# twesterhout/distributed-matvec

Measured on AMD Instinct MI355X. Metric: matvecs/sec, higher is better.
Workload: dtype f64; 1 GPU; heisenberg_chain_32: y <- H x, 601080390 basis states, 9927521280 off-diagonal non-zeros, f64 vectors, sigma/x/y resident in HBM; partitions=1, partitioning=single, exchange=none, kernel=direct-pull+staged, x=u(hash(sigma, 42)) - 0.5, exchange_bytes_per_matvec=0

## Files before the change

distributed-matvec_amd/_lib.py:

```python
from __future__ import annotations

import ctypes as C
import os

_HERE = os.path.dirname(os.path.abspath(__file__))
LIB_PATH = os.path.join(_HERE, os.environ.get("LS_AMD_LIB", "libls_amd.so"))

c_u64p = C.POINTER(C.c_uint64)
c_i64p = C.POINTER(C.c_int64)
c_f64p = C.POINTER(C.c_double)
c_intp = C.POINTER(C.c_int)


class ChplExternalArray(C.Structure):

    _fields_ = [("elts", C.c_void_p), ("num_elts", C.c_uint64), ("freer", C.c_void_p)]


class LsHsBasis(C.Structure):

    _fields_ = [
        ("number_sites", C.c_int),
        ("number_particles", C.c_int),
        ("number_up", C.c_int),
# ... 224 lines not shown
        "ls_amd_repl_plan": (vp, [vp]),
        "ls_amd_repl_exchange_bytes": (C.c_int64, [vp]),
        "ls_amd_repl_x_in_bytes": (C.c_int64, [vp]),
        "ls_amd_enumerate_states": (C.c_int, [bp, C.c_int, C.POINTER(vp), C.POINTER(vp), c_i64p, vp]),
        "ls_amd_gather": (C.c_int, [C.c_int64, vp, C.c_int, C.c_int, vp, vp, vp]),
        "ls_amd_mask_counts": (C.c_int, [C.c_int64, vp, C.c_int, c_i64p, vp]),
        "ls_amd_block_to_hashed": (C.c_int, [C.c_int64, vp, C.c_int, C.c_int, vp, C.POINTER(vp), vp]),
        "ls_amd_hashed_to_block": (C.c_int, [C.c_int64, vp, C.c_int, C.c_int, C.POINTER(vp), vp, vp]),
        "ls_amd_basis_group_order": (C.c_int, [bp]),
        "ls_amd_basis_apply_group_element": (C.c_uint64, [bp, C.c_int, C.c_uint64]),
        "ls_amd_basis_group_character": (C.c_int, [bp, C.c_int, c_f64p, c_f64p]),
        "ls_amd_test_tilemap": (C.c_int64, [C.c_int64, C.c_int, C.c_int64, C.POINTER(C.POINTER(C.c_uint64))]),
        "ls_amd_test_window_find": (C.c_int, [C.POINTER(C.c_uint64), C.c_int, C.c_uint64]),
        "ls_amd_test_nw_find": (C.c_int, [C.POINTER(C.c_uint64), C.c_int, C.c_uint64]),
        "ls_amd_test_chain_near_table": (C.c_int, [C.c_int, C.c_int, C.POINTER(C.c_int16)]),
        "ls_amd_test_rep_trivial_dihedral": (C.c_uint64, [C.c_uint64, C.c_int, C.c_int, C.c_int]),
        "ls_amd_bench_k4": (C.c_int, [C.c_int, C.c_int, C.c_int, C.c_int, C.c_int64, vp, vp, vp]),
        "ls_amd_test_free": (None, [vp]),
        "ls_amd_test_translation_cosets": (C.c_int, [bp, C.POINTER(C.c_int)]),
        "ls_amd_test_rep_by_cosets": (C.c_uint64, [bp, C.c_uint64]),
        "ls_amd_test_d4_mask": (C.c_int, [bp]),
        "ls_amd_test_gtab_bits": (C.c_int, [C.c_int, C.c_int64]),
        "ls_amd_test_gtab_build": (C.c_int, [C.c_int, C.c_int, C.c_int64, C.POINTER(C.c_uint64), C.POINTER(C.c_uint32), C.POINTER(C.POINTER(C.c_uint64))]),
        "ls_amd_test_gtab_find": (C.c_int64, [C.c_int, C.c_int, C.POINTER(C.c_uint64), C.c_uint64]),
        "ls_amd_test_primme_comminfo_offset": (C.c_int, []),
        "ls_amd_test_primme_sumtype_offset": (C.c_int, []),
        "ls_amd_test_primme_nlocal_offset": (C.c_int, []),
        "ls_amd_test_primme_matrix_offset": (C.c_int, []),
        "ls_hs_init": (None, []),
        "ls_hs_exit": (None, []),
# ... 84 lines not shown
```

distributed-matvec_amd/csrc/host.c:

```c
#define _GNU_SOURCE
#include <math.h>
#include <pthread.h>
#include <stdarg.h>
#include <stdio.h>
#include <stdlib.h>
#include <string.h>

#include "../../include/ls_amd.h"
#include "../../include/ls_chpl.h"
#include "../../include/ls_hs.h"
#include "lsk.h"

static __thread char g_last_error[1024] = "";
static ls_amd_error_handler g_handler = NULL;

static int set_error(char const *fmt, ...) {
    va_list ap;
    va_start(ap, fmt);
    vsnprintf(g_last_error, sizeof(g_last_error), fmt, ap);
    va_end(ap);
    return -1;
}
static int dev_error(void) { return set_error("%s", lsk_last_error()); }
int ls_amd_internal_error(char const *fmt, ...) {
// ... 1561 lines not shown
    void *d_tilemap;
    int has_pairs;
    int has_push_staged;
    int one_rank_full_basis;
    lsk_pairplan pairs;
    void *d_pair_recs, *d_rank_low, *d_pair_binom, *d_states32, *d_pair_rows, *d_pair_sites;
    int global_index;
    int has_hubbard;
    lsk_hubbard hubbard;
    void *d_hub[6];
    int has_chain;
    int chain_cached;
    void *d_chain_cache;
    int chain_wide;
    uint64_t *d_chain_rec;
    double chain_v[2];
    int64_t chain_row0;
    void *d_htab;
    uint32_t *d_slot_of;
    int htab_bits;
    void *d_xs;
    int pull_halo;
    int idx_mode;
    struct ls_amd_gtab *gtab;
    uint64_t *d_vtab;
    int64_t row_g0;
    lsk_pullbuf pbuf;
    int64_t split_rows;
    int64_t split_active;
    int slot_cache, slot_cache_valid;
// ... 533 lines not shown
    int const L = NBITS(op->basis);
    int const inv = op->basis->spin_inversion != 0;
    if (inv && (pl->dbs.proj != LSK_PROJ_INVERSION || pl->family != FAMILY_DIRECT_PULL || (L & 1) || BEXT(op->basis)->hamming_weight != L / 2)) return 0;
    if (L > 64 || (!inv && pl->dbs.proj != LSK_PROJ_NONE) ||
        !ext->is_real || !ext->is_hermitian || ext->runs.n_runs <= 0 || ext->n_diag <= 0)
        return 0;
    int extra = 0;
    if (inv) for (int q = 0; q < ext->runs.n_runs; ++q) if (ext->runs.lo0[q] + ext->runs.cnt[q] - 1 == L - 2) extra = 1;
    if (ext->n_groups - ext->runs.n_run_groups + extra > 2) return 0;
    for (int g = ext->runs.n_run_groups; g < ext->n_groups; ++g) {
        lsk_group const *G = &ext->groups[g];
        if (G->fast != LSK_GROUP_EXCHANGE || G->v_im != 0.0 || __builtin_popcountll(G->x) != 2) return 0;
    }
    return 1;
}
static int setup_chain(ls_amd_plan *pl, lsk_index index, int64_t n, uint64_t const *d_reps, void *stream) {
    struct ls_amd_operator_ext const *ext = OEXT(pl->op);
    int nc = ext->n_groups - ext->runs.n_run_groups;
    int const Ls = NBITS(pl->op->basis);
    int const inv = pl->dbs.proj == LSK_PROJ_INVERSION;
    uint64_t const top = 1ULL << (Ls - 1);
    uint64_t cx[3];
    double cv[3];
    int k = 0;
    if (inv)
        for (int q = 0; q < pl->dop.runs.n_runs; ++q)
            if (pl->dop.runs.lo0[q] + pl->dop.runs.cnt[q] - 1 == Ls - 2) {
                cx[k] = 3ULL << (Ls - 2);
                cv[k++] = pl->dop.runs.v_re[q] * (double)pl->op->basis->spin_inversion;
                if (--pl->dop.runs.cnt[q] == 0) {
// ... 36 lines not shown
        pl->chain_v[1] = nc > 1 ? cv[1] : 0.0;
    }
    if (build_tilemap(pl, n, lsk_chain_tile_rows(pl->cplx)) != 0) return -1;
    if (!pl->cplx && NBITS(pl->op->basis) <= 32 && !pl->chain_wide && n > 0) {
        void *q;
        if (lsk_malloc(&q, sizeof(uint64_t) * (size_t)n) != 0) {
            if (pl->d_chain_cache) { lsk_free(pl->d_chain_cache); pl->d_chain_cache = NULL; }
            if (pl->d_tilemap) { lsk_free(pl->d_tilemap); pl->d_tilemap = NULL; memset(&pl->tilemap, 0, sizeof(pl->tilemap)); }
            pl->chain_cached = 0;
            return 0;
        }
        pl->d_chain_rec = (uint64_t *)q;
        DEV(lsk_chain_pack(n, d_reps, pl->chain_cached ? pl->d_chain_cache : NULL, (uint64_t *)q, stream));
        DEV(lsk_sync(stream));
        if (pl->chain_cached <= 1 && pl->d_chain_cache) { lsk_free(pl->d_chain_cache); pl->d_chain_cache = NULL; }
    }
    pl->has_chain = 1;
    return 0;
}

static int pair_cmp(void const *pa, void const *pb) {
    lsk_pair const *a = (lsk_pair const *)pa, *b = (lsk_pair const *)pb;
    int const ca = a->j < 11 ? 0 : (a->i < 11 ? 1 : 2), cb = b->j < 11 ? 0 : (b->i < 11 ? 1 : 2);
    if (ca != cb) return ca - cb;
    if (a->i != b->i) return (int)a->i - (int)b->i;
    return (int)a->j - (int)b->j;
}
static int setup_pairs(ls_amd_plan *pl, int64_t n, uint64_t const *d_reps, void *stream) {
    ls_hs_operator const *op = pl->op;
    struct ls_amd_operator_ext const *ext = OEXT(op);
// ... 814 lines not shown
            if (ps->d_ttab) lsk_free(ps->d_ttab);
            if (ps->d_soff) lsk_free(ps->d_soff);
            if (ps->scatter_gt) ls_amd_internal_gtab_release(ps->scatter_gt);
            free(ps->h_soff);
            free(ps->ttab_first);
            free(ps->send_counts); free(ps->h_beta_off); free(ps->h_val_off);
        }
        free(pl->parts);
    }
    if (pl->d_gtable) lsk_free(pl->d_gtable);
    if (pl->d_row_gidx) lsk_free(pl->d_row_gidx);
    if (pl->d_norms_global) lsk_free(pl->d_norms_global);
    if (pl->d_tilemap) lsk_free(pl->d_tilemap);
    if (pl->d_chain_cache) lsk_free(pl->d_chain_cache);
    if (pl->d_chain_rec) lsk_free(pl->d_chain_rec);
    if (pl->d_pair_recs) lsk_free(pl->d_pair_recs);
    for (int k = 0; k < 6; ++k) if (pl->d_hub[k]) lsk_free(pl->d_hub[k]);
    if (pl->d_pair_rows) lsk_free(pl->d_pair_rows);
    if (pl->d_pair_sites) lsk_free(pl->d_pair_sites);
    if (pl->d_rank_low) lsk_free(pl->d_rank_low);
    if (pl->d_pair_binom) lsk_free(pl->d_pair_binom);
    if (pl->d_states32) lsk_free(pl->d_states32);
    if (pl->d_htab) lsk_free(pl->d_htab);
    if (pl->d_slot_of) lsk_free(pl->d_slot_of);
    if (pl->d_xs) lsk_free(pl->d_xs);
    if (pl->gtab) ls_amd_internal_gtab_release(pl->gtab);
    split_free(pl);
    block_free(pl);
    if (pl->d_send) lsk_free(pl->d_send);
    if (pl->d_cursors) lsk_free(pl->d_cursors);
// ... 141 lines not shown
    if (rc) { lsk_free(nrm); return dev_error(); }
    *d_norms = (double *)nrm;
    return 0;
}

int ls_amd_matvec_replicated(ls_amd_plan *pl, void const *d_x_global, void *d_y_local, void *stream) {
    part_state *ps = &pl->parts[0];
    int slot;
    ls_amd_internal_count_matvec(pl);
    if (pl->family == FAMILY_REPL_DIRECT) {
        int const st = stage_begin(pl, ST_ROWS, stream);
        slot = timing_begin(pl, stream);
        if (pl->has_chain)
            DEV(lsk_chain(pl->dop, pl->dbs, pl->gindex, pl->cplx, pl->chain_wide, pl->d_chain_rec != NULL, pl->tilemap, ps->count,
                          pl->d_chain_rec ? pl->d_chain_rec : ps->d_reps, pl->chain_row0, pl->gindex.count, d_x_global, d_y_local,
                          pl->chain_cached, pl->d_chain_cache, pl->chain_v[0], pl->chain_v[1], stream));
        else
            DEV(lsk_direct_gx(pl->dop, pl->dbs, pl->gindex, pl->cplx, pl->tilemap, ps->d_reps, pl->d_row_gidx, d_x_global,
                          d_y_local, pl->d_err, stream));
        timing_end(pl, slot, stream);
        stage_end(pl, st, stream);
        return 0;
    }
    if (pl->family == FAMILY_REPL_TILE && pl->idx_mode) {
        lsk_pullidx ix;
        ix.tab = pl->gtab->tab;
        ix.perm = pl->gtab->d_perm;
        ix.row_g0 = pl->row_g0;
        ix.vtab = NULL;
        int const st = stage_begin(pl, ST_ROWS, stream);
        slot = timing_begin(pl, stream);
// ... 90 lines not shown
    case FAMILY_DIRECT_PULL:
        if (pl->has_hubbard) return "direct-pull+hubbard";
        return pl->has_chain ? "direct-pull+staged" : pl->has_pairs ? (pl->pairs.sites ? "direct-pull+pairsites" : pl->pairs.rows ? "direct-pull+pairrows" : "direct-pull+pairs") : "direct-pull";
    case FAMILY_TILE_PULL: return pl->idx_mode ? (pl->slot_cache ? "tile-pull+indexed+cached" : (pl->d_vtab ? "tile-pull+values" : "tile-pull+indexed")) : "tile-pull";
    case FAMILY_REPL_DIRECT:
        return pl->has_chain ? "replicated-direct-pull+staged" : "replicated-direct-pull";
    case FAMILY_REPL_TILE: return pl->idx_mode ? (pl->slot_cache ? "replicated-tile-pull+indexed+cached" : "replicated-tile-pull+indexed") : "replicated-tile-pull";
    default: return pl->streams ? "tile+streams" : (pl->has_push_staged ? "tile(one rank: push+staged)" : "tile");
    }
}
int ls_amd_plan_packet_bytes(ls_amd_plan const *pl) { return pl->key_bytes + (pl->cplx ? 16 : 8); }
int ls_amd_plan_row_bytes(ls_amd_plan const *pl) {
    if (pl->has_hubbard) return 0;
    if (pl->has_pairs) return pl->pairs.wide ? 8 : 4;
    if (pl->has_chain) {
        if (pl->d_chain_rec) return 8;
        int const narrow = NBITS(pl->op->basis) <= 32 && !pl->chain_wide;
        return (narrow ? 4 : 8) + pl->chain_cached * (pl->chain_wide ? 8 : 4);
    }
    if (pl->family == FAMILY_TILE_PULL || pl->family == FAMILY_REPL_TILE) return 16;
    return 8;
}
int64_t ls_amd_plan_nnz(ls_amd_plan const *pl) { return pl->nnz; }
int ls_amd_plan_send_counts(ls_amd_plan const *pl, int round, int64_t *counts) {
    if (pl->family != FAMILY_TILE) { for (int d = 0; d < pl->P; ++d) counts[d] = 0; return 0; }
    part_state const *ps = &pl->parts[0];
    if (round < 0 || round >= ps->rounds) return set_error("round out of range");
    memcpy(counts, ps->send_counts + (size_t)round * pl->P, sizeof(int64_t) * pl->P);
    return 0;
}

// ... 240 lines not shown
        }
    } else if (pl->family != FAMILY_DIRECT_PULL) {
        int const st = stage_begin(pl, ST_DIAG, stream);
        for (int p = 0; p < pl->n_local; ++p)
            DEV(lsk_diag(pl->dop, pl->cplx, pl->parts[p].count, pl->parts[p].d_reps, d_x[p], d_y[p], stream));
        stage_end(pl, st, stream);
    }
    if (pl->dop.n_groups == 0 && pl->family != FAMILY_DIRECT_PULL) return 0;
    if (pl->family != FAMILY_TILE) {
        part_state *ps = &pl->parts[0];
        int const st = stage_begin(pl, ST_ROWS, stream);
        int slot = timing_begin(pl, stream);
        if (pl->has_chain)
            DEV(lsk_chain(pl->dop, pl->dbs, ps->index, pl->cplx, pl->chain_wide, pl->d_chain_rec != NULL, pl->tilemap, ps->count,
                          pl->d_chain_rec ? pl->d_chain_rec : ps->d_reps, 0, ps->count, d_x[0], d_y[0], pl->chain_cached,
                          pl->d_chain_cache, pl->chain_v[0], pl->chain_v[1], stream));
        else if (pl->has_pairs)
            DEV(lsk_pairs(pl->pairs, pl->dbs.hamming_weight, pl->cplx, pl->tilemap, ps->count, d_x[0], d_y[0], stream));
        else if (pl->has_hubbard)
            DEV(lsk_hubbard_apply(pl->hubbard, pl->dop, pl->cplx, pl->tilemap, d_x[0], d_y[0], stream));
        else if (pl->has_push_staged)
            DEV(lsk_push_staged(pl->dop, pl->dbs, ps->index, pl->cplx, pl->tilemap, ps->count, ps->d_reps, d_x[0], d_y[0], pl->d_err, stream));
        else
            DEV(lsk_direct(pl->dop, pl->dbs, ps->index, pl->cplx, pl->family == FAMILY_DIRECT_PULL ? (OEXT(pl->op)->is_hermitian ? 1 : 2) : 0, pl->tilemap, ps->d_reps,
                           d_x[0], d_y[0], pl->d_err, stream));
        timing_end(pl, slot, stream);
        stage_end(pl, st, stream);
        return 0;
    }
    int const P = pl->P;
    if (pl->streams) {
// ... 2537 lines not shown
```

distributed-matvec_amd/csrc/k_rows.hip:

```cpp
#include <hip/hip_runtime.h>
#include "lsk_dev.hpp"

template <bool CPLX>
__global__ __launch_bounds__(kBlock) void k_diag(lsk_runs runs, int n_diag, lsk_term const *__restrict__ diag,
                                                 int64_t n, uint64_t const *__restrict__ reps,
                                                 double const *__restrict__ x, double *__restrict__ y) {
    for (int64_t i = (int64_t)blockIdx.x * kBlock + threadIdx.x; i < n; i += (int64_t)gridDim.x * kBlock) {
        uint64_t a = reps[i];
        double dr, di;
        diag_coeff<uint64_t, false>(runs, n_diag, diag, a, dr, di);
        if (CPLX) {
            double xr = x[2 * i], xi = x[2 * i + 1];
            y[2 * i] = dr * xr - di * xi;
            y[2 * i + 1] = dr * xi + di * xr;
        } else {
            y[i] = dr * x[i];
        }
    }
}

extern "C" int lsk_diag(lsk_operator op, int cplx, int64_t n, uint64_t const *reps, void const *x, void *y,
                        void *stream) {
    if (n == 0 || op.n_diag == 0) return 0;
    dim3 g(grid_for(n)), b(kBlock);
// ... 521 lines not shown
    } else if (cplx) hipLaunchKernelGGL((k_push_t<uint64_t, true, 512>), g, b, 0, (hipStream_t)stream, LSK_PT_ARGS);
    else hipLaunchKernelGGL((k_push_t<uint64_t, false, 1024>), g, b, 0, (hipStream_t)stream, LSK_PT_ARGS);
#undef LSK_PT_ARGS
    LSK_LAUNCH_CHECK();
    return 0;
}

extern "C" int lsk_direct_gx(lsk_operator op, lsk_basis bs, lsk_index ix, int cplx, lsk_tilemap tm, uint64_t const *reps,
                             int64_t const *row_gidx, void const *x_global, void *y, int *d_err, void *stream) {
    return direct_dispatch(op, bs, ix, cplx, 1, tm, reps, x_global, y, d_err, stream, 1, row_gidx);
}

constexpr int kChainHalo = 512;
constexpr int kChainLdsPairs = 12;
constexpr int kChainFar = 12;

__device__ __forceinline__ double cx_load_nt(double const *p) { return __builtin_nontemporal_load(p); }
__device__ __forceinline__ double2 cx_load_nt(double2 const *p) {
    typedef double d2v __attribute__((ext_vector_type(2)));
    const d2v v = __builtin_nontemporal_load(reinterpret_cast<d2v const *>(p));
    return make_double2(v.x, v.y);
}
constexpr int kChainFarC = 6;

template <typename W, typename R, bool CPLX, int TILE, bool REC>
__global__ __launch_bounds__(kBlock, (CPLX || sizeof(R) == 8 ? 5 : (sizeof(W) == 8 ? 6 : 7))) void k_chain_t(lsk_runs runs, int n_diag, lsk_term const *__restrict__ diag,
                                                    int hamming_weight, uint4 const *__restrict__ g_img, int img16, int kc,
                                                    int near_off,
                                                    uint64_t const *__restrict__ tilemap, int64_t slots_per_xcd, int64_t n,
                                                    uint64_t const *__restrict__ reps, void const *__restrict__ x_v,
                                                    void *__restrict__ y_v, int hb, int n_cached,
                                                    R const *__restrict__ cache, double cv0, double cv1, int64_t row0,
                                                    int64_t n_x) {
    typedef typename ChainX<CPLX>::type X;
    typedef WordTraits<W> WT;
    constexpr int NB = ChainTraits<W, R>::NB;
    constexpr int HALO = CPLX ? 256 : kChainHalo;
    constexpr int LDSP = CPLX ? 11 : kChainLdsPairs;
    constexpr int WINDOW = TILE + 2 * HALO + 2;
    constexpr int FAR = CPLX ? kChainFarC : kChainFar;
    constexpr R kNone = ~(R)0;
    X const *__restrict__ x = (X const *)x_v;
    X *__restrict__ y = (X *)y_v;
    const bool extra_stream = kAblate && (n_cached & 0x100);
    const int nt_from = !kAblate ? 99 : ((n_cached & 0x200) ? 20 : ((n_cached & 0x400) ? 0 : 99));
    if (kAblate) n_cached &= 0xff;
    uint64_t ex_next = 0;
    extern __shared__ uint4 s_img[];
    R const *const s_binom = reinterpret_cast<R const *>(s_img);
    uint2 const *const s_near = reinterpret_cast<uint2 const *>(reinterpret_cast<char const *>(s_img) + near_off);
    __shared__ X s_x[WINDOW + 1];
    for (int k = threadIdx.x; k < img16; k += kBlock) s_img[k] = g_img[k];
    (void)NB;
    if (threadIdx.x == 0) s_x[WINDOW] = cx_zero<X>();
    const int xcd = blockIdx.x & 7;
    const int64_t blocks_per_xcd = gridDim.x >> 3;
    const int lane = threadIdx.x & 63;
    tilemap += (int64_t)xcd * slots_per_xcd;
    uint32_t const *__restrict__ reps32 = reinterpret_cast<uint32_t const *>(reps);
    for (int64_t t = blockIdx.x >> 3; t < slots_per_xcd; t += blocks_per_xcd) {
        const uint64_t slot = tilemap[t];
        const int cnt = (int)(slot >> 48);
        if (cnt == 0) continue;
        const int64_t i0 = (int64_t)(slot & 0xffffffffffffULL);
        const int64_t w0 = (row0 + i0 - HALO) & ~(int64_t)1;
        W a_next = 0;
        R t0_next = kNone, t1_next = kNone;
        auto load_row = [&](int64_t row, W &a_out, R &t0_out, R &t1_out) {
            if (REC) {
                const uint64_t rec = __builtin_nontemporal_load(reps + row);
                a_out = (W)(uint32_t)rec;
                t0_out = (R)(uint32_t)(rec >> 32);
                if (n_cached == 0) t0_out = kNone;
            } else {
                if (sizeof(W) == 4) a_out = (W)__builtin_nontemporal_load(reps32 + 2 * row);
                else a_out = (W)__builtin_nontemporal_load(reps + row);
                if (n_cached > 0) t0_out = __builtin_nontemporal_load(cache + row);
            }
            if (n_cached > 1) t1_out = __builtin_nontemporal_load(cache + (size_t)n + (size_t)row);
            if (kAblate && extra_stream) ex_next = __builtin_nontemporal_load(reps + (row < (n >> 1) ? row + (n >> 1) : row - (n >> 1)));
        };
        const int wave0 = (int)(threadIdx.x & ~63u);
        if (wave0 < cnt) {
            const int64_t rr = i0 + ((int)threadIdx.x < cnt ? (int)threadIdx.x : cnt - 1);
            load_row(rr, a_next, t0_next, t1_next);
        }
        __syncthreads();
        if (CPLX) {
            for (int j = threadIdx.x; j < WINDOW; j += kBlock) {
                const int64_t row = w0 + j;
                s_x[j] = (row >= 0 && row < n_x) ? x[row] : cx_zero<X>();
            }
        } else {
            double const *xd = (double const *)x_v;
            double *sd = (double *)s_x;
            for (int j = 2 * threadIdx.x; j < WINDOW; j += 2 * kBlock) {
                const int64_t row = w0 + j;
                double2 v;
                if (row >= 0 && row + 1 < n_x) v = *reinterpret_cast<double2 const *>(xd + row);
                else { v.x = (row >= 0 && row < n_x) ? xd[row] : 0.0; v.y = (row + 1 >= 0 && row + 1 < n_x) ? xd[row + 1] : 0.0; }
                sd[j] = v.x;
                sd[j + 1] = v.y;
            }
        }
        __syncthreads();
        const int own0 = (int)(row0 + i0 - w0);
        X y_pending = cx_zero<X>();
        int64_t i_pending = -1;
#pragma unroll 1
        for (int sub = 0; sub < TILE / kBlock; ++sub) {
            const int r = sub * kBlock + threadIdx.x;
            if (i_pending >= 0) cx_store_nt(y + i_pending, y_pending);
            i_pending = -1;
            const W a = a_next;
            const R t0 = t0_next, t1 = t1_next;
            const uint64_t ex = ex_next;
            if (sub + 1 < TILE / kBlock && (sub + 1) * kBlock + wave0 < cnt) {
                const int64_t in = i0 + (r + kBlock < cnt ? r + kBlock : cnt - 1);
                load_row(in, a_next, t0_next, t1_next);
            }
            if (sub * kBlock + wave0 >= cnt) continue;
            const bool ghost = r >= cnt;
            const int64_t i = i0 + (ghost ? cnt - 1 : r);
            const R ig = (R)(row0 + i);
            X g0 = cx_zero<X>(), g1 = cx_zero<X>();
            if (n_cached > 0) g0 = x[t0 != kNone ? t0 : ig];
            if (n_cached > 1) g1 = x[t1 != kNone ? t1 : ig];
            const int jr = own0 + (int)(i - i0);
            const X xr = s_x[jr];
            double dr, di;
            diag_coeff<W, true>(runs, n_diag, diag, a, dr, di);
            X acc = cx_scale(dr, xr);
            const W tdiff = a ^ (a >> 1);
            const W a0 = readfirstlane_t<W>(a);
            const W adiff = a0 ^ readlane_t<W>(a, 63);
            const int ubit = adiff == 0 ? 0 : (int)(8 * sizeof(W)) - (sizeof(W) == 4 ? __clz((int)(uint32_t)adiff) : __clzll((long long)(uint64_t)adiff));
            const R ig0 = readfirstlane_t<R>(ig);
            const uint32_t dl = (uint32_t)(ig - ig0);
            for (int q = 0; q < runs.n_runs; ++q) {
                const int lo0 = runs.lo0[q];
                int lo_end = lo0 + runs.cnt[q];
                const double vr = runs.v_re[q];
                int k = WT::popc(a & (W)(((uint64_t)1 << lo0) - 1));
                int lo = lo0;
                const int e1 = lo_end < LDSP ? lo_end : LDSP;
                const int near_end = lo0 > e1 ? lo0 : e1;
                int split = hb == 0 ? lo_end : (hb < near_end ? near_end : (hb > lo_end ? lo_end : hb));
                if (hb != 0 && split < ubit) split = ubit < lo_end ? ubit : lo_end;
                const bool uni = split < lo_end;
                unsigned long long m = 0;
                R off = 0;
// ... 79 lines not shown
#pragma unroll 4
                for (; lo < lo_end; ++lo) {
                    const bool bit = (a >> lo) & 1;
                    const bool act = (tdiff >> lo) & 1;
                    const R d = s_binom[lo * kc + k];
                    k += bit ? 1 : 0;
                    R idx = bit ? (R)(ig + d) : (R)(ig - d);
                    idx = act ? idx : ig;
                    cx_fma(act ? vr : 0.0, x[idx], acc);
                }
            }
            cx_fma(t0 != kNone ? cv0 : 0.0, g0, acc);
            cx_fma(t1 != kNone ? cv1 : 0.0, g1, acc);
            if (kAblate && extra_stream && ex == 0x0123456789abcdefULL) cx_fma(1.0, xr, acc);
            y_pending = acc;
            i_pending = ghost ? -1 : i;
        }
        if (i_pending >= 0) cx_store_nt(y + i_pending, y_pending);
    }
}

template <typename W, typename R>
__global__ __launch_bounds__(kBlock) void k_chain_cache(int64_t n, uint64_t const *__restrict__ reps, uint64_t xmask, uint64_t inv_mask,
                                                        int hamming_weight, uint64_t const *__restrict__ g_binom,
                                                        R *__restrict__ out, int *__restrict__ flag) {
    constexpr int NB = ChainTraits<W, R>::NB;
    __shared__ R s_binom[NB * LSK_BINOM_K];
    for (int k = threadIdx.x; k < NB * LSK_BINOM_K; k += blockDim.x) s_binom[k] = (R)g_binom[k];
    __syncthreads();
    for (int64_t i = (int64_t)blockIdx.x * kBlock + threadIdx.x; i < n; i += (int64_t)gridDim.x * kBlock) {
        const W a = (W)reps[i];
        R t = ~(R)0;
        if (WordTraits<W>::popc(a & (W)xmask) == 1) {
// ... 20 lines not shown
    LSK_LAUNCH_CHECK();
    return 0;
}

__global__ __launch_bounds__(kBlock) void k_chain_pack(int64_t n, uint64_t const *__restrict__ reps,
                                                       uint32_t const *__restrict__ cache, uint64_t *__restrict__ out) {
    for (int64_t i = (int64_t)blockIdx.x * kBlock + threadIdx.x; i < n; i += (int64_t)gridDim.x * kBlock)
        out[i] = (uint64_t)(uint32_t)reps[i] | ((uint64_t)(cache ? cache[i] : 0xffffffffu) << 32);
}
extern "C" int lsk_chain_pack(int64_t n, uint64_t const *reps, void const *cache, uint64_t *out, void *stream) {
    if (n == 0) return 0;
    hipLaunchKernelGGL(k_chain_pack, dim3(grid_for(n)), dim3(kBlock), 0, (hipStream_t)stream, n, reps, (uint32_t const *)cache, out);
    LSK_LAUNCH_CHECK();
    return 0;
}

__global__ void k_binom_narrow(uint64_t const *__restrict__ in, uint32_t *__restrict__ out, int n) {
    for (int k = blockIdx.x * blockDim.x + threadIdx.x; k < n; k += gridDim.x * blockDim.x) out[k] = (uint32_t)in[k];
}
template <typename R> static R const *chain_binom(uint64_t const *g_binom, hipStream_t stream);
template <> uint64_t const *chain_binom<uint64_t>(uint64_t const *g_binom, hipStream_t) { return g_binom; }
template <> uint32_t const *chain_binom<uint32_t>(uint64_t const *g_binom, hipStream_t stream) {
    static uint64_t const *src = nullptr;
    static uint32_t *narrow = nullptr;
    static std::mutex lock;
    std::lock_guard<std::mutex> guard(lock);
    if (src != g_binom || !narrow) {
        if (!narrow && hipMalloc((void **)&narrow, sizeof(uint32_t) * 64 * LSK_BINOM_K) != hipSuccess) return nullptr;
        hipLaunchKernelGGL(k_binom_narrow, dim3(4), dim3(kBlock), 0, stream, g_binom, narrow, 64 * LSK_BINOM_K);
        src = g_binom;
// ... 50 lines not shown
            if (rsize == 4) reinterpret_cast<uint32_t *>(img.data())[n * kc + k] = (uint32_t)C[n][k];
            else reinterpret_cast<uint64_t *>(img.data())[n * kc + k] = C[n][k];
        }
    if (chain_near_fill(C, elem, ldsp, reinterpret_cast<int16_t *>(img.data() + near_off)) != 0) return -1;
    ChainImage c = {rsize, rows, kc, elem, ldsp, device, nullptr, bytes, near_off};
    if (hipMalloc((void **)&c.dev, (size_t)bytes) != hipSuccess) { snprintf(g_err, sizeof(g_err), "chain_lds_image: no device memory"); return -1; }
    if (hipMemcpy(c.dev, img.data(), (size_t)bytes, hipMemcpyHostToDevice) != hipSuccess) { (void)hipFree(c.dev); snprintf(g_err, sizeof(g_err), "chain_lds_image: copy failed"); return -1; }
    cache.push_back(c);
    *out = c;
    return 0;
}

template <typename W, typename R, bool CPLX, int TILE, bool REC>
static int launch_chain(lsk_operator op, lsk_basis bs, lsk_index ix, lsk_tilemap tm, int64_t n, uint64_t const *reps,
                        int64_t row0, int64_t n_x, void const *x, void *y, int n_cached, void const *cache, double cv0,
                        double cv1, void *stream) {
    int64_t gb = tm.slots_per_xcd * 8;
    ChainImage img;
    if (chain_lds_image((int)sizeof(R), ChainTraits<W, R>::NB, bs.hamming_weight, CPLX ? 16 : 8, CPLX ? 11 : kChainLdsPairs, &img) != 0) return -1;
    hipLaunchKernelGGL((k_chain_t<W, R, CPLX, TILE, REC>), dim3((unsigned)gb), dim3(kBlock), (size_t)img.bytes, (hipStream_t)stream, op.runs,
                       op.n_diag, op.diag, bs.hamming_weight, img.dev, img.bytes / 16, img.kc, img.near_off, tm.entries, tm.slots_per_xcd, n, reps, x, y,
                       kChainLdsPairs, n_cached | ((kAblate && (bs.debug_ablate & 128)) ? 0x100 : 0) | ((kAblate && (bs.debug_ablate & 4096)) ? 0x200 : 0) |
                           ((kAblate && (bs.debug_ablate & 8192)) ? 0x400 : 0), (R const *)cache, cv0, cv1, row0, n_x);
    LSK_LAUNCH_CHECK();
    return 0;
}

extern "C" int lsk_chain_tile_rows(int cplx) { return cplx ? 512 : 1024; }

extern "C" int lsk_chain(lsk_operator op, lsk_basis bs, lsk_index ix, int cplx, int wide_ranks, int fused_records, lsk_tilemap tm,
                         int64_t n, uint64_t const *reps, int64_t row0, int64_t n_x, void const *x, void *y, int n_cached,
                         void const *cache, double cv0, double cv1, void *stream) {
    if (n == 0 || tm.slots_per_xcd == 0) return 0;
    const bool narrow = bs.number_sites <= 32 && !wide_ranks;
#define LSK_CHAIN_ARGS op, bs, ix, tm, n, reps, row0, n_x, x, y, n_cached, cache, cv0, cv1, stream
    if (fused_records) {
        if (!narrow || cplx) { snprintf(g_err, sizeof(g_err), "lsk_chain: fused records need 32-bit states and ranks and f64 vectors"); return -1; }
        return launch_chain<uint32_t, uint32_t, false, 1024, true>(LSK_CHAIN_ARGS);
    }
    if (narrow) {
        if (!cplx) { snprintf(g_err, sizeof(g_err), "lsk_chain: 32-bit states and ranks with f64 vectors run on fused records (lsk_chain_pack)"); return -1; }
        return launch_chain<uint32_t, uint32_t, true, 512, false>(LSK_CHAIN_ARGS);
    }
    if (!wide_ranks) return cplx ? launch_chain<uint64_t, uint32_t, true, 512, false>(LSK_CHAIN_ARGS) : launch_chain<uint64_t, uint32_t, false, 1024, false>(LSK_CHAIN_ARGS);
    return cplx ? launch_chain<uint64_t, uint64_t, true, 512, false>(LSK_CHAIN_ARGS) : launch_chain<uint64_t, uint64_t, false, 1024, false>(LSK_CHAIN_ARGS);
#undef LSK_CHAIN_ARGS
}

constexpr int kPairLowBits = 11;
constexpr int kPairHalo = 512;
// ... 463 lines not shown
```

distributed-matvec_amd/csrc/lsk.h:

```cpp
#ifndef LSK_H
#define LSK_H

#include <stddef.h>
#include <stdint.h>

#ifdef __cplusplus
extern "C" {
#endif

#define LSK_BENES_STAGES 11
#define LSK_BINOM_K 34
#define LSK_MAX_PARTS 256

typedef struct lsk_term {
    double v_re, v_im;
    uint64_t m, r, s;
} lsk_term;

enum { LSK_GROUP_GENERIC = 0, LSK_GROUP_EXCHANGE = 1,
       LSK_GROUP_HOP_LO = 2, LSK_GROUP_HOP_HI = 3 };

typedef struct lsk_group {
    uint64_t x;
    double v_re, v_im;
// ... 149 lines not shown
int lsk_event_create(void **ev);
int lsk_event_destroy(void *ev);
int lsk_event_record(void *ev, void *stream);
int lsk_event_elapsed_ms(void *start, void *stop, float *ms);

int lsk_fill_random(int64_t n, uint64_t const *states, uint64_t seed, int cplx, void *out, void *stream);

int lsk_diag(lsk_operator op, int cplx, int64_t n, uint64_t const *reps, void const *x, void *y,
             void *stream);
int lsk_direct_validate(lsk_operator op, lsk_basis bs, lsk_index ix, int64_t n, uint64_t const *reps, int *d_err, void *stream);
int lsk_direct(lsk_operator op, lsk_basis bs, lsk_index ix, int cplx, int pull, lsk_tilemap tm,
               uint64_t const *reps, void const *x, void *y, int *d_err, void *stream);
int lsk_chain_tile_rows(int cplx);
int lsk_chain(lsk_operator op, lsk_basis bs, lsk_index ix, int cplx, int wide_ranks, int fused_records, lsk_tilemap tm,
              int64_t n, uint64_t const *reps, int64_t row0, int64_t n_x, void const *x, void *y, int n_cached,
              void const *cache, double cv0, double cv1, void *stream);
#define LSK_MAX_PAIRS 128
#define LSK_PAIR_KC 20
typedef struct lsk_pair {
    uint8_t i, j, pad[6];
    double v;
    double vz;
} lsk_pair;
typedef struct lsk_pair_row {
    uint64_t between;
    double v, vz;
    int i, j;
} lsk_pair_row;
#define LSK_PAIR_SITE_MAX_DEGREE 8
#define LSK_PAIR_SITE_MAX_CLASSES 64
typedef struct lsk_pairplan {
// ... 17 lines not shown
typedef struct lsk_species {
    int64_t n;
    int deg;
    uint32_t const *words;
    uint32_t const *rank;
    double const *coef;
} lsk_species;
typedef struct lsk_hubbard {
    int L, cplx_coef;
    lsk_species up, dn;
} lsk_hubbard;
int lsk_hubbard_apply(lsk_hubbard hb, lsk_operator op, int cplx, lsk_tilemap tm, void const *x, void *y, void *stream);
int lsk_narrow_states(int64_t n, uint64_t const *reps, uint32_t *out, void *stream);

int lsk_chain_pack(int64_t n, uint64_t const *reps, void const *cache, uint64_t *out, void *stream);
int lsk_chain_cache(lsk_basis bs, lsk_index ix, int64_t n, uint64_t const *reps, uint64_t xmask, void *out, int wide_ranks,
                    int *d_flag, void *stream);
int lsk_tile(lsk_operator op, lsk_basis bs, lsk_index ix, int cplx, int count_only, int P, int me,
             int64_t row0, int64_t row1, uint64_t const *reps, double const *norms, void const *x,
             void *y, unsigned long long *d_cursors, lsk_round_layout const *d_layout, void *d_send,
             unsigned long long *d_counts, int *d_err, void *stream);
int lsk_tile_wv_max_parts(void);
int lsk_tile_wv(lsk_operator op, lsk_basis bs, lsk_index ix, lsk_gdir gd, int cplx, int count_only, int P, int me,
                int64_t row0, int64_t row1, uint64_t const *reps, double const *norms, void const *x, void *y,
                uint32_t *d_wtab, lsk_round_layout const *d_layout, void *d_send, int *d_err, lsk_gtab own_gt, void *stream);
int lsk_tile_st_max_classes(void);
int lsk_tile_st(lsk_operator op, lsk_gdir gd, uint64_t const *d_binom, int cplx, int count_only, int P, int S, int tile_rows,
                int64_t row0, int64_t row1, uint64_t const *reps, void const *x, uint32_t *d_ttab,
                lsk_round_layout const *d_layout, void *d_send, int *d_err, void *stream);
typedef struct lsk_wsrc {
// ... 290 lines not shown
```

include/ls_amd.h:

```cpp
#ifndef LS_AMD_H
#define LS_AMD_H

#include "ls_hs.h"

#ifdef __cplusplus
extern "C" {
#endif

typedef enum { LS_AMD_F64 = 0, LS_AMD_C128 = 1 } ls_amd_dtype;

typedef enum {
    LS_AMD_MODE_AUTO = 0,
    LS_AMD_MODE_PUSH = 1,
    LS_AMD_MODE_PULL = 2
} ls_amd_mode;

typedef struct ls_amd_plan ls_amd_plan;

char const *ls_amd_last_error(void);
typedef void (*ls_amd_error_handler)(char const *message);
void ls_amd_set_error_handler(ls_amd_error_handler handler);

int ls_amd_device_count(void);
int ls_amd_set_device(int device);
// ... 232 lines not shown
                                   uint64_t *x, uint64_t *s);

int ls_amd_basis_group_order(ls_hs_basis const *basis);
int ls_amd_basis_fermion_signs(ls_hs_basis const *basis);
int ls_amd_test_fermion_sign(ls_hs_basis const *basis, int element, uint64_t state, int table);
int ls_amd_basis_spin_flip(ls_hs_basis const *basis);
int ls_amd_test_group_element_kind(ls_hs_basis const *basis, int element);
uint64_t ls_amd_basis_apply_group_element(ls_hs_basis const *basis, int element, uint64_t state);
int ls_amd_basis_group_character(ls_hs_basis const *basis, int element, double *re, double *im);

int64_t ls_amd_test_tilemap(int64_t n, int tile_rows, int64_t chunk, uint64_t **entries);
void ls_amd_test_free(void *p);
int ls_amd_test_window_find(uint64_t const *reps, int n, uint64_t key);
int ls_amd_test_nw_find(uint64_t const *reps, int n, uint64_t key);
int ls_amd_test_chain_near_table(int elem, int ldsp, int16_t *out);
uint64_t ls_amd_test_rep_trivial_dihedral(uint64_t a, int L, int inv, int reflect);
int ls_amd_bench_k4(int L, int inv, int reflect, int variant, int64_t n, uint64_t const *d_reps, uint64_t *d_out, void *stream);
int ls_amd_test_translation_cosets(ls_hs_basis const *basis, int *n_cosets);
uint64_t ls_amd_test_rep_by_cosets(ls_hs_basis const *basis, uint64_t state);
int ls_amd_test_d4_mask(ls_hs_basis const *basis);
int ls_amd_test_gtab_bits(int L, int64_t n);
int ls_amd_test_gtab_build(int L, int bbits, int64_t n, uint64_t const *reps, uint32_t const *payload, uint64_t **entries);
int64_t ls_amd_test_gtab_find(int L, int bbits, uint64_t const *entries, uint64_t key);
int ls_amd_test_primme_comminfo_offset(void);
int ls_amd_test_primme_sumtype_offset(void);
int ls_amd_test_primme_nlocal_offset(void);
int ls_amd_test_primme_matrix_offset(void);

#ifdef __cplusplus
}
// ... 3 lines not shown
```

Before: 132.0 matvecs/s.

## Replace per-row chain state loads with per-wave compressed headers

Adds a setup kernel that, for each 64-row wave whose states share the same bits above bit 12, stores one 8-byte header: the high bits plus the index into a 4096-entry table of low-12-bit words sorted by popcount, and a base rank for the cached far neighbour. The chain kernel then rebuilds each row's state from that table plus the header instead of streaming an 8-byte record or state per row, and computes the cached neighbour index arithmetically. Waves whose rows don't fit this pattern fall back to per-row loads. The intent is to cut per-row HBM traffic for the state stream, at the cost of extra table lookups, readlane ops and a more complex setup path.

Result: faster. 143.9 matvecs/s (median of 6 runs) (+9.0%).

```diff
diff --git a/distributed-matvec_amd/_lib.py b/distributed-matvec_amd/_lib.py
--- a/distributed-matvec_amd/_lib.py
+++ b/distributed-matvec_amd/_lib.py
@@ -262,6 +262,7 @@
         "ls_amd_test_window_find": (C.c_int, [C.POINTER(C.c_uint64), C.c_int, C.c_uint64]),
         "ls_amd_test_nw_find": (C.c_int, [C.POINTER(C.c_uint64), C.c_int, C.c_uint64]),
         "ls_amd_test_chain_near_table": (C.c_int, [C.c_int, C.c_int, C.POINTER(C.c_int16)]),
+        "ls_amd_test_chain_wave_tables": (C.c_int, [C.c_int, C.POINTER(C.c_uint16), C.POINTER(C.c_uint16), C.POINTER(C.c_int)]),
         "ls_amd_test_rep_trivial_dihedral": (C.c_uint64, [C.c_uint64, C.c_int, C.c_int, C.c_int]),
         "ls_amd_bench_k4": (C.c_int, [C.c_int, C.c_int, C.c_int, C.c_int, C.c_int64, vp, vp, vp]),
         "ls_amd_test_free": (None, [vp]),
diff --git a/distributed-matvec_amd/csrc/host.c b/distributed-matvec_amd/csrc/host.c
--- a/distributed-matvec_amd/csrc/host.c
+++ b/distributed-matvec_amd/csrc/host.c
@@ -1599,6 +1599,8 @@
     void *d_chain_cache;
     int chain_wide;
     uint64_t *d_chain_rec;
+    void *d_chain_wave;
+    int chain_row_bytes;
     double chain_v[2];
     int64_t chain_row0;
     void *d_htab;
@@ -2162,6 +2164,58 @@
     }
     return 1;
 }
+static void chain_wave_tables(int low_site, uint16_t *U, uint16_t *Rg, int *class_off) {
+    int pos[13];
+    uint16_t rank_in[4096];
+    memset(class_off, 0, sizeof(int) * 14);
+    for (int w = 0; w < 4096; ++w) ++class_off[__builtin_popcount(w) + 1];
+    for (int k = 0; k < 13; ++k) { class_off[k + 1] += class_off[k]; pos[k] = class_off[k]; }
+    for (int w = 0; w < 4096; ++w) {
+        int const k = __builtin_popcount(w);
+        rank_in[w] = (uint16_t)(pos[k] - class_off[k]);
+        U[pos[k]++] = (uint16_t)w;
+    }
+    for (int w = 0; w < 4096; ++w) Rg[w] = low_site >= 0 ? rank_in[w ^ (1 << low_site)] : 0;
+}
+int ls_amd_test_chain_wave_tables(int low_site, uint16_t *U, uint16_t *Rg, int *class_off) {
+    if (low_site >= 12) return set_error("ls_amd_test_chain_wave_tables: the low site lies below bit 12");
+    chain_wave_tables(low_site, U, Rg, class_off);
+    return 0;
+}
+static int setup_chain_headers(ls_amd_plan *pl, lsk_index index, int64_t n, uint64_t const *d_reps, int nc, uint64_t xmask, void *stream) {
+    int const L = NBITS(pl->op->basis);
+    char const *e = getenv("LS_AMD_CHAIN_RECORDS");
+    int headed = !(e && atoi(e) != 0) && L >= 13 && L <= 32 && pl->dbs.proj == LSK_PROJ_NONE && pl->chain_row0 == 0 &&
+                 pl->family == FAMILY_DIRECT_PULL && pl->dbs.hamming_weight >= 0 && nc <= 1;
+    int lo = -1, hi = -1;
+    if (headed && nc == 1) {
+        lo = __builtin_ctzll(xmask);
+        hi = 63 - __builtin_clzll(xmask);
+        if (lo >= 12 || hi < 12) { headed = 0; lo = hi = -1; }
+    }
+    int const words = lsk_chain_words();
+    int64_t const n_hdr = (n + 63) / 64;
+    uint16_t U[4096], Rg[4096];
+    int class_off[14];
+    uint32_t *tab = (uint32_t *)malloc(sizeof(uint32_t) * (size_t)words);
+    if (!tab) return set_error("out of memory");
+    chain_wave_tables(headed ? lo : -1, U, Rg, class_off);
+    for (int t = 0; t < words; ++t) tab[t] = (uint32_t)U[t] | ((uint32_t)Rg[U[t]] << 16) | (lo >= 0 ? (((uint32_t)U[t] >> lo) & 1u) << 31 : 0u);
+    size_t const tab_bytes = sizeof(uint32_t) * (size_t)words, hdr_bytes = 8 * (size_t)n_hdr;
+    void *q;
+    if (lsk_malloc(&q, tab_bytes + hdr_bytes + 8) != 0) { free(tab); return 1; }
+    unsigned long long plain = 0;
+    unsigned long long *d_plain = (unsigned long long *)((char *)q + tab_bytes + hdr_bytes);
+    int const rc = lsk_h2d(q, tab, tab_bytes) || lsk_h2d(d_plain, &plain, 8) ||
+                   lsk_chain_headers(pl->dbs, index, n, d_reps, headed, hi, (char *)q + tab_bytes, d_plain, stream) || lsk_sync(stream) ||
+                   lsk_d2h(&plain, d_plain, 8);
+    free(tab);
+    if (rc) { lsk_free(q); return dev_error(); }
+    pl->d_chain_wave = q;
+    int const rec = pl->cplx ? 4 + 4 * nc : 8;
+    pl->chain_row_bytes = headed ? (int)((8 * (uint64_t)n_hdr + 64 * (uint64_t)rec * (uint64_t)plain + (uint64_t)n - 1) / (uint64_t)n) : rec;
+    return 0;
+}
 static int setup_chain(ls_amd_plan *pl, lsk_index index, int64_t n, uint64_t const *d_reps, void *stream) {
     struct ls_amd_operator_ext const *ext = OEXT(pl->op);
     int nc = ext->n_groups - ext->runs.n_run_groups;
@@ -2228,6 +2282,17 @@
         DEV(lsk_chain_pack(n, d_reps, pl->chain_cached ? pl->d_chain_cache : NULL, (uint64_t *)q, stream));
         DEV(lsk_sync(stream));
         if (pl->chain_cached <= 1 && pl->d_chain_cache) { lsk_free(pl->d_chain_cache); pl->d_chain_cache = NULL; }
+    }
+    if (NBITS(pl->op->basis) <= 32 && !pl->chain_wide && n > 0) {
+        int const rc = setup_chain_headers(pl, index, n, d_reps, pl->chain_cached, pl->chain_cached > 0 ? cx[0] : 0, stream);
+        if (rc < 0) return -1;
+        if (rc > 0) {
+            if (pl->d_chain_rec) { lsk_free(pl->d_chain_rec); pl->d_chain_rec = NULL; }
+            if (pl->d_chain_cache) { lsk_free(pl->d_chain_cache); pl->d_chain_cache = NULL; }
+            if (pl->d_tilemap) { lsk_free(pl->d_tilemap); pl->d_tilemap = NULL; memset(&pl->tilemap, 0, sizeof(pl->tilemap)); }
+            pl->chain_cached = 0;
+            return 0;
+        }
     }
     pl->has_chain = 1;
     return 0;
@@ -3072,6 +3137,7 @@
     if (pl->d_tilemap) lsk_free(pl->d_tilemap);
     if (pl->d_chain_cache) lsk_free(pl->d_chain_cache);
     if (pl->d_chain_rec) lsk_free(pl->d_chain_rec);
+    if (pl->d_chain_wave) lsk_free(pl->d_chain_wave);
     if (pl->d_pair_recs) lsk_free(pl->d_pair_recs);
     for (int k = 0; k < 6; ++k) if (pl->d_hub[k]) lsk_free(pl->d_hub[k]);
     if (pl->d_pair_rows) lsk_free(pl->d_pair_rows);
@@ -3243,7 +3309,7 @@
         if (pl->has_chain)
             DEV(lsk_chain(pl->dop, pl->dbs, pl->gindex, pl->cplx, pl->chain_wide, pl->d_chain_rec != NULL, pl->tilemap, ps->count,
                           pl->d_chain_rec ? pl->d_chain_rec : ps->d_reps, pl->chain_row0, pl->gindex.count, d_x_global, d_y_local,
-                          pl->chain_cached, pl->d_chain_cache, pl->chain_v[0], pl->chain_v[1], stream));
+                          pl->chain_cached, pl->d_chain_cache, pl->chain_v[0], pl->chain_v[1], pl->d_chain_wave, stream));
         else
             DEV(lsk_direct_gx(pl->dop, pl->dbs, pl->gindex, pl->cplx, pl->tilemap, ps->d_reps, pl->d_row_gidx, d_x_global,
                           d_y_local, pl->d_err, stream));
@@ -3364,7 +3430,7 @@
     if (pl->has_hubbard) return 0;
     if (pl->has_pairs) return pl->pairs.wide ? 8 : 4;
     if (pl->has_chain) {
-        if (pl->d_chain_rec) return 8;
+        if (pl->d_chain_wave) return pl->chain_row_bytes;
         int const narrow = NBITS(pl->op->basis) <= 32 && !pl->chain_wide;
         return (narrow ? 4 : 8) + pl->chain_cached * (pl->chain_wide ? 8 : 4);
     }
@@ -3635,7 +3701,7 @@
         if (pl->has_chain)
             DEV(lsk_chain(pl->dop, pl->dbs, ps->index, pl->cplx, pl->chain_wide, pl->d_chain_rec != NULL, pl->tilemap, ps->count,
                           pl->d_chain_rec ? pl->d_chain_rec : ps->d_reps, 0, ps->count, d_x[0], d_y[0], pl->chain_cached,
-                          pl->d_chain_cache, pl->chain_v[0], pl->chain_v[1], stream));
+                          pl->d_chain_cache, pl->chain_v[0], pl->chain_v[1], pl->d_chain_wave, stream));
         else if (pl->has_pairs)
             DEV(lsk_pairs(pl->pairs, pl->dbs.hamming_weight, pl->cplx, pl->tilemap, ps->count, d_x[0], d_y[0], stream));
         else if (pl->has_hubbard)
diff --git a/distributed-matvec_amd/csrc/k_rows.hip b/distributed-matvec_amd/csrc/k_rows.hip
--- a/distributed-matvec_amd/csrc/k_rows.hip
+++ b/distributed-matvec_amd/csrc/k_rows.hip
@@ -559,6 +559,7 @@
 constexpr int kChainHalo = 512;
 constexpr int kChainLdsPairs = 12;
 constexpr int kChainFar = 12;
+constexpr uint32_t kChainWords = 4096;
 
 __device__ __forceinline__ double cx_load_nt(double const *p) { return __builtin_nontemporal_load(p); }
 __device__ __forceinline__ double2 cx_load_nt(double2 const *p) {
@@ -574,9 +575,9 @@
                                                     int near_off,
                                                     uint64_t const *__restrict__ tilemap, int64_t slots_per_xcd, int64_t n,
                                                     uint64_t const *__restrict__ reps, void const *__restrict__ x_v,
-                                                    void *__restrict__ y_v, int hb, int n_cached,
+                                                    void *__restrict__ y_v, int n_cached,
                                                     R const *__restrict__ cache, double cv0, double cv1, int64_t row0,
-                                                    int64_t n_x) {
+                                                    int64_t n_x, uint32_t const *__restrict__ wave_plan) {
     typedef typename ChainX<CPLX>::type X;
     typedef WordTraits<W> WT;
     constexpr int NB = ChainTraits<W, R>::NB;
@@ -585,6 +586,7 @@
     constexpr int WINDOW = TILE + 2 * HALO + 2;
     constexpr int FAR = CPLX ? kChainFarC : kChainFar;
     constexpr R kNone = ~(R)0;
+    constexpr int hb = kChainLdsPairs;
     X const *__restrict__ x = (X const *)x_v;
     X *__restrict__ y = (X *)y_v;
     const bool extra_stream = kAblate && (n_cached & 0x100);
@@ -603,6 +605,8 @@
     const int lane = threadIdx.x & 63;
     tilemap += (int64_t)xcd * slots_per_xcd;
     uint32_t const *__restrict__ reps32 = reinterpret_cast<uint32_t const *>(reps);
+    constexpr bool HDR = REC || (CPLX && sizeof(W) == 4 && sizeof(R) == 4);
+    constexpr int NSUB = TILE / kBlock;
     for (int64_t t = blockIdx.x >> 3; t < slots_per_xcd; t += blocks_per_xcd) {
         const uint64_t slot = tilemap[t];
         const int cnt = (int)(slot >> 48);
@@ -616,7 +620,6 @@
                 const uint64_t rec = __builtin_nontemporal_load(reps + row);
                 a_out = (W)(uint32_t)rec;
                 t0_out = (R)(uint32_t)(rec >> 32);
-                if (n_cached == 0) t0_out = kNone;
             } else {
                 if (sizeof(W) == 4) a_out = (W)__builtin_nontemporal_load(reps32 + 2 * row);
                 else a_out = (W)__builtin_nontemporal_load(reps + row);
@@ -626,9 +629,21 @@
             if (kAblate && extra_stream) ex_next = __builtin_nontemporal_load(reps + (row < (n >> 1) ? row + (n >> 1) : row - (n >> 1)));
         };
         const int wave0 = (int)(threadIdx.x & ~63u);
+        uint32_t hq = ~0u;
+        if (HDR) {
+            const uint32_t hw = 2 * (uint32_t)(i0 >> 6) + 2 * ((threadIdx.x >> 6) + (uint32_t)(lane % NSUB) * (kBlock / 64)) + (lane / NSUB) % 2;
+            if (((int64_t)(hw >> 1) << 6) < n) hq = wave_plan[kChainWords + hw];
+        }
+        auto fetch_row = [&](int s, int64_t row) {
+            if (HDR) {
+                const uint32_t ti = (uint32_t)__builtin_amdgcn_readlane((int)hq, s) & (kChainWords - 1u);
+                if (ti != kChainWords - 1u) { a_next = (W)wave_plan[ti + lane]; return; }
+            }
+            load_row(row, a_next, t0_next, t1_next);
+        };
         if (wave0 < cnt) {
             const int64_t rr = i0 + ((int)threadIdx.x < cnt ? (int)threadIdx.x : cnt - 1);
-            load_row(rr, a_next, t0_next, t1_next);
+            fetch_row(0, rr);
         }
         __syncthreads();
         if (CPLX) {
@@ -651,35 +666,48 @@
         __syncthreads();
         const int own0 = (int)(row0 + i0 - w0);
         X y_pending = cx_zero<X>();
-        int64_t i_pending = -1;
+        int r_pending = -1;
 #pragma unroll 1
         for (int sub = 0; sub < TILE / kBlock; ++sub) {
             const int r = sub * kBlock + threadIdx.x;
-            if (i_pending >= 0) cx_store_nt(y + i_pending, y_pending);
-            i_pending = -1;
-            const W a = a_next;
-            const R t0 = t0_next, t1 = t1_next;
+            if (r_pending >= 0) cx_store_nt(y + i0 + r_pending, y_pending);
+            r_pending = -1;
+            W a = a_next;
+            R t0 = t0_next;
+            const R t1 = t1_next;
             const uint64_t ex = ex_next;
             if (sub + 1 < TILE / kBlock && (sub + 1) * kBlock + wave0 < cnt) {
                 const int64_t in = i0 + (r + kBlock < cnt ? r + kBlock : cnt - 1);
-                load_row(in, a_next, t0_next, t1_next);
+                fetch_row(sub + 1, in);
             }
             if (sub * kBlock + wave0 >= cnt) continue;
             const bool ghost = r >= cnt;
             const int64_t i = i0 + (ghost ? cnt - 1 : r);
             const R ig = (R)(row0 + i);
-            X g0 = cx_zero<X>(), g1 = cx_zero<X>();
-            if (n_cached > 0) g0 = x[t0 != kNone ? t0 : ig];
-            if (n_cached > 1) g1 = x[t1 != kNone ? t1 : ig];
+            W a0;
+            int ubit;
+            const uint32_t h0 = HDR ? (uint32_t)__builtin_amdgcn_readlane((int)hq, sub) : ~0u;
+            if (HDR && (h0 & (kChainWords - 1u)) != kChainWords - 1u) {
+                const uint32_t word = (uint32_t)a;
+                a0 = (W)(h0 & ~(kChainWords - 1u));
+                a = a0 | (W)(word & (kChainWords - 1u));
+                ubit = 0;
+                const uint32_t h1 = (uint32_t)__builtin_amdgcn_readlane((int)hq, NSUB + sub);
+                t0 = (int32_t)(word ^ h1) < 0 ? (R)((h1 & 0x7fffffffu) + ((word >> 16) & 0x7fffu)) : kNone;
+            } else {
+                a0 = readfirstlane_t<W>(a);
+                const W adiff = a0 ^ readlane_t<W>(a, 63);
+                ubit = adiff == 0 ? 0 : (int)(8 * sizeof(W)) - (sizeof(W) == 4 ? __clz((int)(uint32_t)adiff) : __clzll((long long)(uint64_t)adiff));
+            }
             const int jr = own0 + (int)(i - i0);
             const X xr = s_x[jr];
+            X g0 = n_cached > 0 ? xr : cx_zero<X>(), g1 = n_cached > 1 ? xr : cx_zero<X>();
+            if (t0 != kNone) g0 = x[t0];
+            if (n_cached > 1 && t1 != kNone) g1 = x[t1];
             double dr, di;
             diag_coeff<W, true>(runs, n_diag, diag, a, dr, di);
             X acc = cx_scale(dr, xr);
             const W tdiff = a ^ (a >> 1);
-            const W a0 = readfirstlane_t<W>(a);
-            const W adiff = a0 ^ readlane_t<W>(a, 63);
-            const int ubit = adiff == 0 ? 0 : (int)(8 * sizeof(W)) - (sizeof(W) == 4 ? __clz((int)(uint32_t)adiff) : __clzll((long long)(uint64_t)adiff));
             const R ig0 = readfirstlane_t<R>(ig);
             const uint32_t dl = (uint32_t)(ig - ig0);
             for (int q = 0; q < runs.n_runs; ++q) {
@@ -789,9 +817,9 @@
             cx_fma(t1 != kNone ? cv1 : 0.0, g1, acc);
             if (kAblate && extra_stream && ex == 0x0123456789abcdefULL) cx_fma(1.0, xr, acc);
             y_pending = acc;
-            i_pending = ghost ? -1 : i;
-        }
-        if (i_pending >= 0) cx_store_nt(y + i_pending, y_pending);
+            r_pending = ghost ? -1 : r;
+        }
+        if (r_pending >= 0) cx_store_nt(y + i0 + r_pending, y_pending);
     }
 }
 
@@ -842,6 +870,50 @@
     LSK_LAUNCH_CHECK();
     return 0;
 }
+
+__global__ __launch_bounds__(kBlock) void k_chain_headers(int64_t n, uint64_t const *__restrict__ reps, int hamming_weight, int high_site,
+                                                          uint64_t const *__restrict__ g_binom, uint2 *__restrict__ out,
+                                                          unsigned long long *__restrict__ n_plain) {
+    const int64_t n_hdr = (n + 63) >> 6;
+    for (int64_t w = (int64_t)blockIdx.x * kBlock + threadIdx.x; w < n_hdr; w += (int64_t)gridDim.x * kBlock) {
+        uint2 h = make_uint2(~0u, ~0u);
+        const uint32_t first = (uint32_t)reps[w << 6];
+        if ((w << 6) + 63 < n && ((first ^ (uint32_t)reps[(w << 6) + 63]) >> 12) == 0) {
+            const uint32_t high = first & ~(kChainWords - 1u), low = first & (kChainWords - 1u);
+            const int kl = __popc(low);
+            uint32_t ti = (uint32_t)rank_combinadic_w<uint32_t, uint64_t>(low, g_binom);
+            for (int k = 0; k < kl; ++k) ti += (uint32_t)g_binom[12 * LSK_BINOM_K + k];
+            uint32_t base = 0;
+            if (high_site >= 0) {
+                const uint32_t hbit = (high >> high_site) & 1u;
+                const int kp = hbit ? kl + 1 : kl - 1;
+                if (kp >= 0 && kp <= 12 && kp <= hamming_weight)
+                    base = (uint32_t)rank_combinadic_w<uint32_t, uint64_t>((high ^ (1u << high_site)) | ((1u << kp) - 1u), g_binom);
+                base |= hbit << 31;
+            }
+            h = make_uint2(high | ti, base);
+        } else
+            atomicAdd(n_plain, 1ULL);
+        out[w] = h;
+    }
+}
+extern "C" int lsk_chain_headers(lsk_basis bs, lsk_index ix, int64_t n, uint64_t const *reps, int headed, int high_site, void *out,
+                                 unsigned long long *d_n_plain, void *stream) {
+    if (n == 0) return 0;
+    if (!headed) {
+        if (hipMemsetAsync(out, 0xff, 8 * (size_t)((n + 63) >> 6), (hipStream_t)stream) != hipSuccess) { snprintf(g_err, sizeof(g_err), "lsk_chain_headers: memset failed"); return -1; }
+        return 0;
+    }
+    if (bs.number_sites > 32 || bs.number_sites < 13 || bs.hamming_weight < 0 || high_site >= bs.number_sites || (high_site >= 0 && high_site < 12)) {
+        snprintf(g_err, sizeof(g_err), "lsk_chain_headers: plan out of range");
+        return -1;
+    }
+    hipLaunchKernelGGL(k_chain_headers, dim3(grid_for((n + 63) >> 6)), dim3(kBlock), 0, (hipStream_t)stream, n, reps, bs.hamming_weight,
+                       high_site, ix.binom, (uint2 *)out, d_n_plain);
+    LSK_LAUNCH_CHECK();
+    return 0;
+}
+extern "C" int lsk_chain_words(void) { return (int)kChainWords; }
 
 __global__ void k_binom_narrow(uint64_t const *__restrict__ in, uint32_t *__restrict__ out, int n) {
     for (int k = blockIdx.x * blockDim.x + threadIdx.x; k < n; k += gridDim.x * blockDim.x) out[k] = (uint32_t)in[k];
@@ -922,14 +994,15 @@
 template <typename W, typename R, bool CPLX, int TILE, bool REC>
 static int launch_chain(lsk_operator op, lsk_basis bs, lsk_index ix, lsk_tilemap tm, int64_t n, uint64_t const *reps,
                         int64_t row0, int64_t n_x, void const *x, void *y, int n_cached, void const *cache, double cv0,
-                        double cv1, void *stream) {
+                        double cv1, void const *wave_plan, void *stream) {
     int64_t gb = tm.slots_per_xcd * 8;
     ChainImage img;
     if (chain_lds_image((int)sizeof(R), ChainTraits<W, R>::NB, bs.hamming_weight, CPLX ? 16 : 8, CPLX ? 11 : kChainLdsPairs, &img) != 0) return -1;
     hipLaunchKernelGGL((k_chain_t<W, R, CPLX, TILE, REC>), dim3((unsigned)gb), dim3(kBlock), (size_t)img.bytes, (hipStream_t)stream, op.runs,
                        op.n_diag, op.diag, bs.hamming_weight, img.dev, img.bytes / 16, img.kc, img.near_off, tm.entries, tm.slots_per_xcd, n, reps, x, y,
-                       kChainLdsPairs, n_cached | ((kAblate && (bs.debug_ablate & 128)) ? 0x100 : 0) | ((kAblate && (bs.debug_ablate & 4096)) ? 0x200 : 0) |
-                           ((kAblate && (bs.debug_ablate & 8192)) ? 0x400 : 0), (R const *)cache, cv0, cv1, row0, n_x);
+                       n_cached | ((kAblate && (bs.debug_ablate & 128)) ? 0x100 : 0) | ((kAblate && (bs.debug_ablate & 4096)) ? 0x200 : 0) |
+                           ((kAblate && (bs.debug_ablate & 8192)) ? 0x400 : 0), (R const *)cache, cv0, cv1, row0, n_x,
+                       (uint32_t const *)wave_plan);
     LSK_LAUNCH_CHECK();
     return 0;
 }
@@ -938,10 +1011,11 @@
 
 extern "C" int lsk_chain(lsk_operator op, lsk_basis bs, lsk_index ix, int cplx, int wide_ranks, int fused_records, lsk_tilemap tm,
                          int64_t n, uint64_t const *reps, int64_t row0, int64_t n_x, void const *x, void *y, int n_cached,
-                         void const *cache, double cv0, double cv1, void *stream) {
+                         void const *cache, double cv0, double cv1, void const *wave_plan, void *stream) {
     if (n == 0 || tm.slots_per_xcd == 0) return 0;
     const bool narrow = bs.number_sites <= 32 && !wide_ranks;
-#define LSK_CHAIN_ARGS op, bs, ix, tm, n, reps, row0, n_x, x, y, n_cached, cache, cv0, cv1, stream
+    if ((wave_plan != nullptr) != narrow) { snprintf(g_err, sizeof(g_err), "lsk_chain: 32-bit states and ranks come with wave headers, the other plans without"); return -1; }
+#define LSK_CHAIN_ARGS op, bs, ix, tm, n, reps, row0, n_x, x, y, n_cached, cache, cv0, cv1, wave_plan, stream
     if (fused_records) {
         if (!narrow || cplx) { snprintf(g_err, sizeof(g_err), "lsk_chain: fused records need 32-bit states and ranks and f64 vectors"); return -1; }
         return launch_chain<uint32_t, uint32_t, false, 1024, true>(LSK_CHAIN_ARGS);
diff --git a/distributed-matvec_amd/csrc/lsk.h b/distributed-matvec_amd/csrc/lsk.h
--- a/distributed-matvec_amd/csrc/lsk.h
+++ b/distributed-matvec_amd/csrc/lsk.h
@@ -187,7 +187,7 @@
 int lsk_chain_tile_rows(int cplx);
 int lsk_chain(lsk_operator op, lsk_basis bs, lsk_index ix, int cplx, int wide_ranks, int fused_records, lsk_tilemap tm,
               int64_t n, uint64_t const *reps, int64_t row0, int64_t n_x, void const *x, void *y, int n_cached,
-              void const *cache, double cv0, double cv1, void *stream);
+              void const *cache, double cv0, double cv1, void const *wave_plan, void *stream);
 #define LSK_MAX_PAIRS 128
 #define LSK_PAIR_KC 20
 typedef struct lsk_pair {
@@ -235,6 +235,9 @@
 int lsk_narrow_states(int64_t n, uint64_t const *reps, uint32_t *out, void *stream);
 
 int lsk_chain_pack(int64_t n, uint64_t const *reps, void const *cache, uint64_t *out, void *stream);
+int lsk_chain_headers(lsk_basis bs, lsk_index ix, int64_t n, uint64_t const *reps, int headed, int high_site, void *out,
+                      unsigned long long *d_n_plain, void *stream);
+int lsk_chain_words(void);
 int lsk_chain_cache(lsk_basis bs, lsk_index ix, int64_t n, uint64_t const *reps, uint64_t xmask, void *out, int wide_ranks,
                     int *d_flag, void *stream);
 int lsk_tile(lsk_operator op, lsk_basis bs, lsk_index ix, int cplx, int count_only, int P, int me,
diff --git a/include/ls_amd.h b/include/ls_amd.h
--- a/include/ls_amd.h
+++ b/include/ls_amd.h
@@ -270,6 +270,7 @@
 int ls_amd_test_window_find(uint64_t const *reps, int n, uint64_t key);
 int ls_amd_test_nw_find(uint64_t const *reps, int n, uint64_t key);
 int ls_amd_test_chain_near_table(int elem, int ldsp, int16_t *out);
+int ls_amd_test_chain_wave_tables(int low_site, uint16_t *U, uint16_t *Rg, int *class_off);
 uint64_t ls_amd_test_rep_trivial_dihedral(uint64_t a, int L, int inv, int reflect);
 int ls_amd_bench_k4(int L, int inv, int reflect, int variant, int64_t n, uint64_t const *d_reps, uint64_t *d_out, void *stream);
 int ls_amd_test_translation_cosets(ls_hs_basis const *basis, int *n_cosets);
```
